# INDA23PlusPlus/isaklm-raytracer

Measured on AMD Instinct MI355X. Metric: Msamples/sec (W×H×spp/s) at 1920×1080; achieved HBM GB/s vs peak, higher is better.
Workload: dtype f32

## Files before the change

### isaklm-raytracer_amd/csrc/wavefront.hip

```cpp
#include <hip/hip_runtime.h>

#include <stdio.h>
#include <stdlib.h>
#include <string.h>
#include <time.h>

#include <algorithm>
#include <chrono>
#include <atomic>
#include <map>
#include <mutex>
#include <thread>
#include <vector>

#include "bvh_trace.h"
#include "rt_kernels.h"

using namespace rtk;

#define WF_BLOCK 256
#ifndef WF_TBLOCK
#define WF_TBLOCK 256
#endif
static_assert(WF_BLOCK % WF_TBLOCK == 0 && WF_TBLOCK % 64 == 0, "WF_TBLOCK must divide WF_BLOCK in whole waves");
// ... 1561 lines not shown
    uint32_t *fetch = st.counts + 4;
    const int limit = fr.max_depth > 0 ? fr.max_depth : RT_WATCHDOG_BOUNCES;

    PathRegs p;
    p.slot = 0;
    p.ro = p.rd = rt_v3(0, 0, 0);
    CoopRay r;
    coop_idle(r);
    int hit = -1;
    float bx = 0.0f, by = 0.0f, bz = 0.0f;
    bool active = false;
    bool exhausted = lane >= ppw;
    bool pending = false;
    while (true) {
        const bool need = !active && !exhausted;
        const unsigned long long m = __ballot(need);
        if (m) {
            const int leader = __ffsll((long long)m) - 1;
            uint32_t base = 0;
            if (lane == leader) base = atomicAdd(fetch, (uint32_t)__popcll(m));
            base = __shfl(base, leader);
            if (need) {
                const uint32_t e = base + (uint32_t)__popcll(m & ((1ull << lane) - 1ull));
                if (e >= n) {
                    exhausted = true;
                } else {
                    active = true;
                    first_ray(st, fr, st.q_slot[q][e], p);
                    if (COUNT) c.v[RT_CNT_RAY]++;
                    if (!coop_begin(sc, r, p.ro, p.rd)) {
                        pending = true;
                        hit = -1;
                    }
                }
            }
        }
        while (pending) {
            pending = false;
            if (shade_step<COUNT>(sc, fr, cam, p, hit, bx, by, bz, limit, c)) {
                if (COUNT) c.v[RT_CNT_RAY]++;
                if (!coop_begin(sc, r, p.ro, p.rd)) {
                    pending = true;
                    hit = -1;
                }
            } else {
                store_regs(st, fr, p);
                active = false;
            }
        }
        const unsigned long long lm = __ballot(r.live);
        if (!lm) {
            if (__all(exhausted)) break;
            continue;
        }
        if (__popcll(lm) <= wide) {
            const WideLds W{s_wide + wave * WIDE_CAP, WIDE_CAP, wkey, reinterpret_cast<float *>(wkey + 1), w.mark};
            for (unsigned long long mm = lm; mm; mm &= mm - 1) {
                const int owner = __ffsll((long long)mm) - 1;
                const int ot = wave * 64 + owner;
                const Stack<WF_LDS_STACK> so{s_node + ot, s_entry + ot, WF_BLOCK,
                                             st.spill + blockIdx.x * WF_BLOCK + ot, st.spill_threads};
                int t;
                float x, y, z;
                wide_resume<COUNT>(sc, r, owner, so, W, t, x, y, z, c);
                if (lane == owner) {
                    hit = t;
                    bx = x;
                    by = y;
                    bz = z;
                    r.live = false;
                    pending = true;
                }
            }
            continue;
        }
        if (coop_round<COUNT>(sc, r, stk, w, cap, postpone, hit, bx, by, bz, c)) pending = true;
    }
    if (COUNT) {
        flush_counters(c, fr.counters);
        flush_finish_counters(c, fr.counters);
    }
}

template <bool COUNT>
__global__ void __launch_bounds__(WF_BLOCK, WF_LONG_WAVES) wf_long(RtDevScene sc, RtDevFrame fr, RtDevCamera cam, WfState st,
                                                    int final_slice)
{
    __shared__ __attribute__((aligned(16))) WideItem s_wide[(WF_BLOCK / 64) * WIDE_CAP];
    static_assert(WSM_LDS_BYTES <= WIDE_CAP * sizeof(WideItem), "the wide s_min query's lists reuse the wave's frontier");
    static_assert(WSM_KD_STACK * 8 <= 128 * sizeof(int), "the bounded KD phase's stack reuses the wave's chunk_owner marks");
    __shared__ unsigned long long s_key[(WF_BLOCK / 64) * 4];
    __shared__ __attribute__((aligned(8))) int s_mark[2 * WF_BLOCK];
    if (WF_LONG_PRIO > 0) __builtin_amdgcn_s_setprio(WF_LONG_PRIO);
    const int lane = __lane_id();
    const int wave = threadIdx.x >> 6;
    const WideLds W{s_wide + wave * WIDE_CAP, WIDE_CAP, s_key + wave * 4,
                    reinterpret_cast<float *>(s_key + wave * 4 + 1), s_mark + wave * 128};
    Cnt c;
    if (COUNT) c.zero();
    const int limit = fr.max_depth > 0 ? fr.max_depth : RT_WATCHDOG_BOUNCES;
    uint32_t *const reserved = st.long_ctr, *const claimed = st.long_ctr + 1, *const running = st.long_ctr + 3;
    const bool persist = st.fin_live != nullptr;
    unsigned long long t_idle = __builtin_amdgcn_s_memrealtime();
    unsigned long long t_net = t_idle;
    unsigned long long t_pub = 0;
    uint32_t n_idle = 0, n_net = 0, n_pub = 0, n_start = 0;
    uint32_t r_seen = 0, e_pub = 0xffffffffu;
    while (true) {
        uint32_t e = 0, slot = 0;
        RtF4 ro4{0, 0, 0, 0}, rd4{0, 0, 0, 0};
        int quit = 0;
        if (lane == 0) {
            while (true) {
                const unsigned long long now = __builtin_amdgcn_s_memrealtime();
                ++n_idle;
                ++n_net;
                const uint32_t fl = persist ? __hip_atomic_load(st.fin_live, __ATOMIC_RELAXED, __HIP_MEMORY_SCOPE_AGENT) : 0u;
                const bool unstarted = persist && !(fl & WF_FIN_STARTED);
                const bool producing = persist && !unstarted && (fl & ~WF_FIN_STARTED) != 0u;
                const bool others = __hip_atomic_load(running, __ATOMIC_RELAXED, __HIP_MEMORY_SCOPE_AGENT) != 0u;
                const bool chain_open =
                    persist && __hip_atomic_load(st.chain_flag, __ATOMIC_RELAXED, __HIP_MEMORY_SCOPE_AGENT) != 0u;
                if (persist && !producing && !unstarted) __builtin_amdgcn_fence(__ATOMIC_ACQUIRE, "agent");
                e = __hip_atomic_load(claimed, __ATOMIC_RELAXED, __HIP_MEMORY_SCOPE_AGENT);
                const uint32_t rw = __hip_atomic_load(reserved, __ATOMIC_RELAXED, __HIP_MEMORY_SCOPE_AGENT);
                const bool closed = (rw & WF_LONG_CLOSED) != 0u;
                const uint32_t r = rw & ~WF_LONG_CLOSED;
                const bool flowing = r != r_seen;
                if (flowing) {
                    r_seen = r;
                    t_idle = now;
                    n_idle = 0;
                }
                if (flowing || producing || others) {
                    t_net = now;
                    n_net = 0;
                }
                const bool window_over = (now - t_idle > WF_LONG_CHAIN_IDLE || n_idle > WF_LONG_CHAIN_TRIPS) && !others;
                const bool done = persist && (closed || (!producing && !unstarted && (!chain_open || window_over)));
                if (st.debug_quit) {
                    quit = 2;
                    break;
                }
                if (e < r) {
                    const uint32_t k = e % st.long_cap;
                    const unsigned long long v =
                        __hip_atomic_load(st.long_ent + k, __ATOMIC_RELAXED, __HIP_MEMORY_SCOPE_AGENT);
                    if ((uint32_t)(v >> 32) == e + 1u) {
                        __builtin_amdgcn_fence(__ATOMIC_ACQUIRE, "agent");
                        ro4 = ldf4(st.long_ray + 2 * (size_t)k);
                        rd4 = ldf4(st.long_ray + 2 * (size_t)k + 1);
                        slot = (uint32_t)v;
                        asm volatile("s_waitcnt vmcnt(0)" ::: "memory");
                        uint32_t expect = e;
                        if (__hip_atomic_compare_exchange_strong(claimed, &expect, e + 1u, __ATOMIC_RELAXED,
                                                                 __ATOMIC_RELAXED, __HIP_MEMORY_SCOPE_AGENT)) {
                            __hip_atomic_fetch_add(running, 1u, __ATOMIC_RELAXED, __HIP_MEMORY_SCOPE_AGENT);
                            break;
                        }
                        continue;
                    }
                    if (e != e_pub) {
                        e_pub = e;
                        t_pub = now;
                        n_pub = 0;
                    } else if (now - t_pub > WF_LONG_PUBLISH_WAIT || ++n_pub > WF_LONG_PUBLISH_TRIPS) {
                        quit = 2;
                        break;
                    }
                } else {
                    if (persist ? done : (final_slice || !others)) {
                        quit = 1;
                        break;
                    }
                    if (unstarted && !closed && ++n_start > WF_LONG_START_TRIPS) {
                        uint32_t x = r;
                        if (__hip_atomic_compare_exchange_strong(reserved, &x, r | WF_LONG_CLOSED, __ATOMIC_RELAXED,
                                                                 __ATOMIC_RELAXED, __HIP_MEMORY_SCOPE_AGENT)) {
                            atomicAdd(fr.dev_stats + RT_DEV_LONG_CLOSED, 1ull);
                            quit = 1;
                            break;
                        }
                        continue;
                    }
                }
                if (now - t_net > WF_LONG_IDLE || n_net > WF_LONG_IDLE_TRIPS) {
                    quit = e < r ? 2 : 1;
                    break;
                }
                __builtin_amdgcn_s_sleep(16);
            }
            if (!quit) asm volatile("s_waitcnt vmcnt(0)" ::: "memory");
            if (quit == 2) atomicAdd(fr.dev_stats + RT_DEV_LONG_QUIT, 1ull);
        }
        if (__builtin_amdgcn_readfirstlane(quit)) break;
        e = (uint32_t)__builtin_amdgcn_readfirstlane((int)e);
        PathRegs p;
        p.slot = 0;
        p.ro = p.rd = rt_v3(0, 0, 0);
        if (lane == 0) {
            load_regs(st, fr, slot, p);
            p.ro = ld3(ro4);
            p.rd = ld3(rd4);
        }
        int want = 0;
        uint32_t ret_e = 0;
        const unsigned long long t_claim = __builtin_amdgcn_s_memrealtime();
        uint32_t bounces = 0;
        while (true) {
            ++bounces;
            int hit = -1;
            float bx = 0.0f, by = 0.0f, bz = 0.0f;
            CoopRay r;
            coop_idle(r);
            if (lane == 0) {
                if (COUNT) c.v[RT_CNT_RAY]++;
                coop_begin(sc, r, p.ro, p.rd);
            }
            if (__shfl((int)r.live, 0)) {
                const Vec3D o = rt_v3(__shfl(r.o.x, 0), __shfl(r.o.y, 0), __shfl(r.o.z, 0));
                const Vec3D d = rt_v3(__shfl(r.d.x, 0), __shfl(r.d.y, 0), __shfl(r.d.z, 0));
                const float en = __shfl(r.entry, 0), ex = __shfl(r.exit_, 0);
                bool traced = false;
                bool certified = false;
                if (st.long_wide && rt_bounded_ray(o, d, sc.split_vals, sc.split_off)) {
                    float s_min = ex;
                    int tk = -1;
                    traced = wide_smin<COUNT>(sc, o, d, ex, wsm_lds(W.F, W.key, st.long_wide == 2), s_min, tk, c);
                    if (traced && s_min < ex)
                        certified = kd_certified<COUNT>(sc, o, d, en, ex, s_min, tk, hit, bx, by, bz, c, lane == 0);
                    if (traced && s_min < ex && !certified) {
                        LdsStack1 ks{reinterpret_cast<uint2 *>(W.mark)};
                        const int tstar = tk >= 0 ? (int)sc.bvh_bary[tk].tri : -1;
                        hit = kd_bounded_wave<COUNT>(sc, o, d, en, ex, s_min, tstar, bx, by, bz, ks,
                                                     reinterpret_cast<unsigned long long *>(W.F), c);
                    }
                    if (!traced && lane == 0) atomicAdd(fr.dev_stats + RT_DEV_WIDE_OVERFLOW, 1ull);
                }
                if (!traced) {
                    const int nf = !COUNT && sc.kd_grid > 0 ? kd_origin_frontier(sc, o, d, en, ex, W) : 0;
                    if (nf > 0) wide_trace_from<COUNT>(sc, o, d, nf, W, lane == 0, hit, bx, by, bz, c);
                    else wide_trace<COUNT>(sc, o, d, en, ex, W, lane == 0, hit, bx, by, bz, c);
                }
                if (COUNT && lane == 0 && hit >= 0 && !certified) c.cert[1]++;
            }
            want = 0;
            if (lane == 0) {
                want = shade_step<COUNT>(sc, fr, cam, p, hit, bx, by, bz, limit, c) ? 1 : 0;
                if (!want && st.long_return) {
                    while (true) {
                        store_regs(st, fr, p);
                        asm volatile("s_waitcnt vmcnt(0)" ::: "memory");
                        __builtin_amdgcn_fence(__ATOMIC_RELEASE, "agent");
                        uint32_t x = RT_PX_OUT;
                        if (__hip_atomic_compare_exchange_strong(st.pxo + p.slot, &x, RT_PX_LONGDONE, __ATOMIC_RELAXED,
                                                                 __ATOMIC_RELAXED, __HIP_MEMORY_SCOPE_AGENT))
                            break;
                        x = __hip_atomic_exchange(st.pxo + p.slot, RT_PX_OUT, __ATOMIC_RELAXED,
                                                  __HIP_MEMORY_SCOPE_AGENT);
                        p.passes_left = (int)(x & RT_PX_PASSES);
                        if (x & RT_PX_PASSES) {
                            atomicAdd(fr.dev_stats + RT_DEV_OWED_PIXELS, 1ull);
                            atomicAdd(fr.dev_stats + RT_DEV_OWED_PASSES, (unsigned long long)(x & RT_PX_PASSES));
                        }
                        const Vec3D fb = fr.fb[p.slot];
                        const float sq = fr.sq[p.slot];
                        const int count = fr.count[p.slot];
                        if (start_sample<COUNT>(fr, cam, (int)p.slot, p.passes_left, p.rng, fb, sq, count, p.ro, p.rd,
                                                c)) {
                            p.T = rt_v3(1.0f, 1.0f, 1.0f);
                            p.L = rt_v3(0.0f, 0.0f, 0.0f);
                            p.inside = false;
                            p.prev_type = PRIMARY;
                            p.depth = 1;
                            p.shadow = false;
                            want = 1;
                            break;
                        }
                    }
                }
                if (want && st.long_return && p.depth == 1 && !p.shadow) {
                    unsigned long long *const ret_word = reinterpret_cast<unsigned long long *>(st.ret_ctr);
                    if (st.linger == 0ull &&
                        __hip_atomic_load(st.chain_flag, __ATOMIC_RELAXED, __HIP_MEMORY_SCOPE_AGENT) != 0u) {
                        want = 2;
                        ret_e = (uint32_t)__hip_atomic_fetch_add(ret_word, 1ull, __ATOMIC_RELAXED, __HIP_MEMORY_SCOPE_AGENT);
                    }
                    unsigned long long w = __hip_atomic_load(ret_word, __ATOMIC_RELAXED, __HIP_MEMORY_SCOPE_AGENT);
                    while (want != 2 && (w >> 32) != 0ull) {
                        if (__hip_atomic_compare_exchange_strong(ret_word, &w, w + 1ull, __ATOMIC_RELAXED,
                                                                 __ATOMIC_RELAXED, __HIP_MEMORY_SCOPE_AGENT)) {
                            want = 2;
                            ret_e = (uint32_t)w;
                            break;
                        }
                    }
                }
            }
            want = __builtin_amdgcn_readfirstlane(want);
            if (want != 1) break;
        }
        if (lane == 0) {
            if (st.long_log && e < 65535u) {
                unsigned long long *L = st.long_log + 4 + 4 * (size_t)e;
                L[0] = t_claim;
                L[1] = __builtin_amdgcn_s_memrealtime();
                L[2] = bounces;
                L[3] = p.slot;
            }
            if (want == 2) {
                store_regs(st, fr, p);
                st.ro[p.slot] = p.ro;
                st.cont[p.slot] = p.rd;
                asm volatile("s_waitcnt vmcnt(0)" ::: "memory");
                __builtin_amdgcn_fence(__ATOMIC_RELEASE, "agent");
                asm volatile("s_waitcnt vmcnt(0)" ::: "memory");
                __hip_atomic_store(st.ret_ring + ret_e % st.long_cap, ((unsigned long long)(ret_e + 1u) << 32) | p.slot,
                                   __ATOMIC_RELAXED, __HIP_MEMORY_SCOPE_AGENT);
            } else if (st.long_return) {
                __hip_atomic_fetch_sub(st.ret_ctr + 3, 1u, __ATOMIC_RELAXED, __HIP_MEMORY_SCOPE_AGENT);
            } else {
                store_regs(st, fr, p);
            }
            __hip_atomic_fetch_sub(running, 1u, __ATOMIC_RELAXED, __HIP_MEMORY_SCOPE_AGENT);
        }
        t_idle = __builtin_amdgcn_s_memrealtime();
        n_idle = 0;
    }
    if (COUNT) {
        flush_counters(c, fr.counters);
        flush_cert_counters(c, fr.dev_stats);
    }
}

void rt_register_shutdown();

namespace {

struct Pipe {
    std::vector<std::pair<float, float>> trace_iv;
    WfState st{};
    hipStream_t stream = nullptr;
    uint32_t *host_count = nullptr;
    hipEvent_t ev[6] = {};
    hipEvent_t join = nullptr;
    hipEvent_t fin_done = nullptr;
    hipEvent_t long_done = nullptr;
    bool joined = false;
    bool long_rec = false;
    RtProfile prof{};
};

struct ChainKey {
    const void *nodes, *bvh, *fb, *sq, *count, *rng;
    int width, height, adaptive, min_samples, max_depth, shard_id, num_shards, long_depth;
    float tolerance;
    RtDevCamera cam;
};

ChainKey chain_key(const RtDevScene &sc, const RtDevFrame &fr, const RtDevCamera &cam, int long_depth)
{
    ChainKey key;
    memset(&key, 0, sizeof key);
    key.nodes = sc.nodes;
    key.bvh = sc.bvh_nodes;
    key.fb = fr.fb;
    key.sq = fr.sq;
    key.count = fr.count;
    key.rng = fr.rng;
    key.width = fr.width;
    key.height = fr.height;
    key.adaptive = fr.adaptive;
    key.min_samples = fr.min_samples;
    key.max_depth = fr.max_depth;
    key.shard_id = fr.shard_id;
    key.num_shards = fr.num_shards;
    key.long_depth = long_depth;
    key.tolerance = fr.tolerance;
    key.cam = cam;
    return key;
}

struct Pending {
    bool on = false;
    int dev = 0;
    RtDevScene sc{};
    RtDevFrame fr{};
    RtDevCamera cam{};
    hipStream_t stream = nullptr;
    int long_depth = 0, debug = 0, calls = 0;
    bool prof = false;
    uint32_t check_mask = 0;
    ChainKey key{};
};

struct Workspace {
    Pending pend;
    size_t slots = 0;
    int grid = 0;
    int spill_pipes = 0;
    void *blob = nullptr;
    Pipe pipe[WF_MAX_PIPES];
    bool streams_ok = false;
    hipEvent_t fork = nullptr, ev0 = nullptr, ev1 = nullptr, fin_ready = nullptr;
    hipEvent_t long_ev = nullptr;
    bool recorded = false;
    uint32_t *fin_live = nullptr;
    uint32_t *heavy_list = nullptr;
    RtF4 *chk = nullptr;
    uint32_t chk_cap = 0;
    uint32_t *chk_ctr = nullptr;
    uint32_t *verify_res = nullptr;
    bool verify_pending = false;
    bool verify_unread = false;
    hipEvent_t verify_ev = nullptr;
// ... 177 lines not shown
        st.cont = (Vec3D *)(b + o_c);
        st.snorm = (Vec3D *)(b + o_n);
        st.rp = (Vec3D *)(b + o_rp);
        st.light = (int *)(b + o_li);
        st.ro = (Vec3D *)(b + o_ro);
        st.e_sh = (uint32_t *)(b + o_es);
        st.e_ext = (uint32_t *)(b + o_ee);
        st.q_slot[0] = (uint32_t *)(b + o_qs0[i]);
        st.q_slot[1] = (uint32_t *)(b + o_qs1[i]);
        st.q_ray[0] = (RtF4 *)(b + o_qr0[i]);
        st.q_ray[1] = (RtF4 *)(b + o_qr1[i]);
        st.hits = (RtF4 *)(b + o_h[i]);
        st.counts = (uint32_t *)(b + o_cnt[i]);
        st.spill = i < spill_pipes ? (uint2 *)(b + o_sp[i]) : nullptr;
        st.spill_threads = (int)spill_threads;
        st.long_ctr = (uint32_t *)(b + o_lc);
        st.long_ent = (unsigned long long *)(b + o_le);
        st.long_ray = (RtF4 *)(b + o_lr);
        st.long_depth = 0;
        st.long_cap = (uint32_t)slots;
        st.long_return = 0;
        st.ret_ring = (unsigned long long *)(b + o_rr);
        st.ret_ctr = (uint32_t *)(b + o_rc);
        st.linger = WF_FIN_LINGER;
        st.pxo = (uint32_t *)(b + o_px);
        st.heavy = (uint8_t *)(b + o_hv);
        st.listed = (uint32_t *)(b + o_ls);
        st.heavy_list = nullptr;
        w.heavy_list = (uint32_t *)(b + o_hl);
        st.heavy_n = (uint32_t *)(b + o_hn);
        st.fin_live = nullptr;
        st.chain_flag = (uint32_t *)(b + o_ctl + 128);
        st.fresh = 0;
        st.fresh_n = 0;
        st.span = nullptr;
        st.call_id = 0;
        st.chk = nullptr;
        st.chk_ctr = nullptr;
        st.chk_mask = 0;
        st.chk_cap = 0;
        st.chk_fault = 0;
        st.debug_quit = 0;
        st.long_wide = 0;
    }
    w.slots = slots;
    w.grid = grid;
    w.spill_pipes = spill_pipes;
    return 0;
}

float elapsed_ms(hipEvent_t a, hipEvent_t b)
{
    float ms = 0.0f;
    return hipEventElapsedTime(&ms, a, b) == hipSuccess ? ms : 0.0f;
}

int launch_verify(Workspace &w, hipStream_t stream)
{
    if (!w.verify_pending || !w.blob) return 0;
    w.verify_pending = false;
    const int blocks = (int)std::min<size_t>((w.slots + WF_BLOCK - 1) / WF_BLOCK, 1024);
    hipLaunchKernelGGL(wf_verify, dim3(blocks), dim3(WF_BLOCK), 0, stream, w.pipe[0].st, (uint32_t)w.slots,
                       w.verify_res, w.last_fr.dev_stats);
    if (hipGetLastError() != hipSuccess) return -1;
    if (hipEventRecord(w.verify_ev, stream) != hipSuccess) return -1;
    w.verify_rec = true;
    w.verify_unread = true;
    return 0;
}

int join_all(Workspace &w, hipStream_t stream)
{
    if (launch_drain(w) != 0) return -1;
    if (w.verify_rec && hipStreamWaitEvent(stream, w.verify_ev, 0) != hipSuccess) return -1;
    for (int pi = 0; pi < WF_MAX_PIPES; ++pi) {
        Pipe &p = w.pipe[pi];
        if (p.joined && hipStreamWaitEvent(stream, p.join, 0) != hipSuccess) return -1;
        if (p.long_rec && hipStreamWaitEvent(stream, p.long_done, 0) != hipSuccess) return -1;
    }
    if (w.recorded && hipStreamWaitEvent(stream, w.long_ev, 0) != hipSuccess) return -1;
    return launch_verify(w, stream);
}

int debug_long_log(Workspace &w, unsigned long long *buf);

int launch_whole_now(Workspace &w, int dev, const RtDevScene &sc, const RtDevFrame &fr, const RtDevCamera &cam,
                     hipStream_t stream, int long_depth, bool prof, bool overlap, uint32_t check_mask, int debug,
                     bool count)
{
    const size_t slots = (size_t)fr.width * fr.height;
    overlap = overlap && !fr.reset;
    if (!w.cus) {
        hipDeviceProp_t prop;
        w.cus = hipGetDeviceProperties(&prop, dev) == hipSuccess && prop.multiProcessorCount > 0
                    ? prop.multiProcessorCount
                    : 256;
    }
    const int grid = w.cus * 4 * WF_FIN_BVH_WAVES / (WF_BLOCK / 64);
    const ChainKey key = chain_key(sc, fr, cam, long_depth);
    const bool chained = overlap && w.chain_open && !fr.reset && memcmp(&key, &w.key, sizeof key) == 0;
    if (!chained && join_all(w, stream) != 0) return -1;
    if (ensure(w, slots, grid, 1) != 0) return -1;
    Pipe &pp = w.pipe[0];
    WfState st = pp.st;
    const int long_return = long_depth > 0 ? 1 : 0;
    st.long_depth = long_depth;
    st.long_return = long_return;
    st.fresh = 1;
    st.fresh_n = (uint32_t)(((fr.width + 15) / 16) * ((fr.height + 15) / 16)) * 256u;
    st.linger = overlap ? 0ull : WF_FIN_LINGER;
    st.chk_mask = check_mask;
    const int par = (int)(w.call_seq & 1);
    if (check_mask != 0xFFFFFFFFu) {
        const unsigned long long per_sample =
            check_mask == 0u ? 2ull * (unsigned long long)(long_depth > 0 ? long_depth : RT_DEEP_PATH) + 2ull : 8ull;
        const unsigned long long want = (unsigned long long)slots * (unsigned long long)fr.passes * per_sample /
                                        ((unsigned long long)check_mask + 1ull);
        uint32_t cap = 1u << 16;
        while (cap < want && cap < WF_CHECK_CAP) cap <<= 1;
        if (cap > w.chk_cap) {
            if (w.chk) {
                if (hipDeviceSynchronize() != hipSuccess) return -1;
                (void)hipFree(w.chk);
                w.chk = nullptr;
                w.chk_cap = 0;
            }
            if (hipMalloc((void **)&w.chk, 2 * (size_t)cap * 3 * sizeof(RtF4)) != hipSuccess) {
                w.chk = nullptr;
                return -1;
            }
            w.chk_cap = cap;
        }
    }
    st.chk = check_mask == 0xFFFFFFFFu ? nullptr : w.chk + 3 * (size_t)w.chk_cap * (size_t)par;
    st.chk_cap = w.chk_cap;
    st.chk_ctr = w.chk_ctr + par;
    st.chk_fault = (debug & RT_DEBUG_CHECK_FAULT) ? 1 : 0;
    st.debug_quit = (debug & RT_DEBUG_LONG_QUIT) ? 1 : 0;
    st.long_wide = sc.bvh_wide ? ((debug & RT_DEBUG_WIDE_CAP1) ? 2 : 1) : 0;
    if ((debug & RT_DEBUG_LONG_LOG) && !w.long_log_buf &&
        hipMalloc((void **)&w.long_log_buf, 8 * 4 * 65536) != hipSuccess) {
        w.long_log_buf = nullptr;
        return -1;
    }
    unsigned long long *const long_log_buf = w.long_log_buf;
    st.long_log = (debug & RT_DEBUG_LONG_LOG) ? long_log_buf : nullptr;
    int fgrid = (int)((slots + WF_BLOCK - 1) / WF_BLOCK);
    const int fmax = long_return ? grid - WF_LONG_BLOCKS : grid;
    fgrid = fgrid > fmax ? fmax : fgrid;
    const uint32_t k = (uint32_t)(w.call_seq % 8);
    st.fin_live = long_return ? w.fin_live + k : nullptr;
    st.call_id = (uint32_t)w.call_seq + 1u;
    if (!chained) {
        if (long_return) {
            if (hipMemsetAsync(st.long_ctr, 0, 256, stream) != hipSuccess) return -1;
            if (hipMemsetAsync(st.long_ent, 0, (size_t)st.long_cap * 8, stream) != hipSuccess) return -1;
            if (hipMemsetAsync(st.ret_ring, 0, (size_t)st.long_cap * 8, stream) != hipSuccess) return -1;
            if (hipMemsetAsync(st.ret_ctr, 0, 256, stream) != hipSuccess) return -1;
        }
        if (st.long_log && hipMemsetAsync(long_log_buf, 0, 8 * 4 * 65536, stream) != hipSuccess) return -1;
    }
    ++w.call_seq;
    const hipStream_t s = pp.stream;
    if (hipEventRecord(w.fork, stream) != hipSuccess || hipStreamWaitEvent(s, w.fork, 0) != hipSuccess) return -1;
    if (hipMemsetAsync(st.counts, 0, 256, s) != hipSuccess) return -1;
    if (st.fin_live && hipMemsetD32Async((hipDeviceptr_t)st.fin_live, (int)(fgrid * (WF_BLOCK / 64)), 1, s) != hipSuccess)
        return -1;
    if (st.chk) {
        if (w.chk_rec[par] && hipStreamWaitEvent(s, w.chk_done[par], 0) != hipSuccess) return -1;
        if (hipMemsetAsync(st.chk_ctr, 0, 4, s) != hipSuccess) return -1;
    }
    if (long_return && hipMemsetD32Async((hipDeviceptr_t)st.chain_flag, overlap ? 1 : 0, 1, s) != hipSuccess) return -1;
    st.span = nullptr;
    if (prof) {
        if (prof_slot(w, s, &st.span, fr.passes) != 0) return -1;
    }
    st.heavy_list = nullptr;
    if (long_return && w.heavy_list && WF_HEAVY_FIRST) {
        st.heavy_list = w.heavy_list;
        if (hipMemsetAsync(st.heavy_n, 0, 4, s) != hipSuccess) return -1;
        hipLaunchKernelGGL(wf_heavy_list, dim3(WF_HEAVY_BLOCKS), dim3(WF_BLOCK), 0, s, fr, st, st.call_id,
                           (uint32_t)WF_HEAVY_SPLIT, 256u);
        hipLaunchKernelGGL(wf_heavy_list, dim3(WF_HEAVY_BLOCKS), dim3(WF_BLOCK), 0, s, fr, st, st.call_id, 1u,
                           (uint32_t)WF_HEAVY_SPLIT);
        if (hipGetLastError() != hipSuccess) return -1;
    }
    if (hipEventRecord(w.fin_ready, s) != hipSuccess) return -1;
    Pipe *lp = long_return ? &w.pipe[1] : nullptr;
    const bool long_first = lp && (debug & RT_DEBUG_SERIAL_LONG_FIRST);
    const bool fin_first = lp && !long_first && (debug & RT_DEBUG_SERIAL_FIN_FIRST);
    auto launch_long = [&]() -> int {
        if (hipStreamWaitEvent(lp->stream, fin_first ? pp.fin_done : w.fin_ready, 0) != hipSuccess) return -1;
        if (count) hipLaunchKernelGGL(wf_long<true>, dim3(WF_LONG_BLOCKS), dim3(WF_BLOCK), 0, lp->stream, sc, fr, cam, st, 1);
        else hipLaunchKernelGGL(wf_long<false>, dim3(WF_LONG_BLOCKS), dim3(WF_BLOCK), 0, lp->stream, sc, fr, cam, st, 1);
        if (hipGetLastError() != hipSuccess) return -1;
        if (hipEventRecord(lp->long_done, lp->stream) != hipSuccess) return -1;
        lp->long_rec = true;
        return 0;
    };
    if (long_first && (launch_long() != 0 || hipStreamWaitEvent(s, lp->long_done, 0) != hipSuccess)) return -1;
    if (count && !(debug & RT_DEBUG_COUNT_LONG_ONLY)) hipLaunchKernelGGL(wf_finish_bvh<true>, dim3(fgrid), dim3(WF_BLOCK), 0, s, sc, fr, cam, st, 0);
    else if (fgrid <= w.cus * WF_FIN_SMALL_WAVES)
        hipLaunchKernelGGL((wf_finish_bvh<false, 1>), dim3(fgrid), dim3(WF_BLOCK), 0, s, sc, fr, cam, st, 0);
    else hipLaunchKernelGGL(wf_finish_bvh<false>, dim3(fgrid), dim3(WF_BLOCK), 0, s, sc, fr, cam, st, 0);
    if (hipGetLastError() != hipSuccess) return -1;
    if (hipEventRecord(pp.fin_done, s) != hipSuccess) return -1;
    if (lp && !long_first && launch_long() != 0) return -1;
    if (st.chk) {
        Pipe &cp = w.pipe[2];
        WfState cs = st;
        cs.spill = cp.st.spill;
        if (!cs.spill) return -1;
        if (hipStreamWaitEvent(cp.stream, pp.fin_done, 0) != hipSuccess) return -1;
        hipLaunchKernelGGL(wf_check, dim3(WF_CHECK_BLOCKS), dim3(WF_BLOCK), 0, cp.stream, sc, cs, fr.dev_stats);
        if (hipGetLastError() != hipSuccess) return -1;
        if (hipEventRecord(w.chk_done[par], cp.stream) != hipSuccess || hipEventRecord(cp.join, cp.stream) != hipSuccess)
            return -1;
        w.chk_rec[par] = true;
        cp.joined = true;
    }
    if (hipEventRecord(pp.join, s) != hipSuccess) return -1;
    pp.joined = true;
    if (!overlap) {
        if (hipStreamWaitEvent(stream, pp.join, 0) != hipSuccess) return -1;
        if (lp && hipStreamWaitEvent(stream, lp->long_done, 0) != hipSuccess) return -1;
    }
    w.chain_open = overlap && long_return;
    w.verify_pending = w.verify_pending || long_return;
    w.key = key;
    w.last_sc = sc;
    w.last_fr = fr;
    w.last_fr.reset = 0;
    w.last_cam = cam;
    w.last_long_depth = long_depth;
    w.last_debug = debug;
    if (debug & RT_DEBUG_CALL_LOG) {
        (void)hipStreamSynchronize(s);
        timespec ts;
        clock_gettime(CLOCK_MONOTONIC, &ts);
        uint32_t lc[4] = {}, rc4[7] = {};
        (void)hipMemcpy(lc, st.long_ctr, sizeof lc, hipMemcpyDeviceToHost);
        (void)hipMemcpy(rc4, st.ret_ctr, sizeof rc4, hipMemcpyDeviceToHost);
        fprintf(stderr,
                "[wf] call %llu%s finisher done t %.4f; long entries %u claimed %u running %u; returns reserved %u "
                "claimed %u, finisher waves alive %u, pixels out %u; owed passes: most %u, pixels %u\n",
                w.call_seq, chained ? " (chained)" : "", ts.tv_sec + ts.tv_nsec * 1e-9, lc[0], lc[1], lc[3], rc4[0],
                rc4[2], rc4[1], rc4[3], rc4[5], rc4[6]);
    }
    if (st.long_log && !overlap) return debug_long_log(w, long_log_buf);
    return 0;
}

int flush_pending(Workspace &w)
{
    if (!w.pend.on) return 0;
    Pending b = w.pend;
    w.pend.on = false;
    return launch_whole_now(w, b.dev, b.sc, b.fr, b.cam, b.stream, b.long_depth, b.prof, true, b.check_mask, b.debug,
                            false);
}

int launch_whole(Workspace &w, int dev, const RtDevScene &sc, const RtDevFrame &fr, const RtDevCamera &cam,
                 hipStream_t stream, int long_depth, bool prof, bool overlap, uint32_t check_mask, int debug,
                 bool count, int coalesce)
{
    const bool can = overlap && !fr.reset && !count && coalesce > 0 && !fr.wave_times &&
                     !(debug & (RT_DEBUG_CALL_LOG | RT_DEBUG_LONG_LOG | RT_DEBUG_SERIAL_LONG_FIRST |
                                RT_DEBUG_SERIAL_FIN_FIRST));
    if (w.pend.on) {
        const ChainKey key = chain_key(sc, fr, cam, long_depth);
        if (can && w.pend.dev == dev && w.pend.stream == stream && w.pend.prof == prof &&
            w.pend.check_mask == check_mask && w.pend.debug == debug && w.pend.sc.nodes == sc.nodes &&
            memcmp(&key, &w.pend.key, sizeof key) == 0 && (long long)w.pend.fr.passes + fr.passes < (1LL << 28)) {
            w.pend.fr.passes += fr.passes;
            ++w.pend.calls;
            return w.pend.fr.passes < coalesce ? 0 : flush_pending(w);
        }
        if (flush_pending(w) != 0) return -1;
    }
    if (can && fr.passes < coalesce) {
        Pending &b = w.pend;
        b.on = true;
        b.dev = dev;
        b.sc = sc;
        b.fr = fr;
        b.cam = cam;
        b.stream = stream;
        b.long_depth = long_depth;
        b.debug = debug;
        b.calls = 1;
        b.prof = prof;
        b.check_mask = check_mask;
        b.key = chain_key(sc, fr, cam, long_depth);
        return 0;
    }
    return launch_whole_now(w, dev, sc, fr, cam, stream, long_depth, prof, overlap, check_mask, debug, count);
}

int launch_drain(Workspace &w)
{
    if (flush_pending(w) != 0) return -1;
    if (!w.chain_open) return 0;
    w.chain_open = false;
    const RtDevFrame &fr = w.last_fr;
    const size_t slots = (size_t)fr.width * fr.height;
    Pipe &pp = w.pipe[0];
    WfState st = pp.st;
    st.long_depth = w.last_long_depth;
    st.long_return = 1;
    st.fresh = 1;
    st.fresh_n = 0;
    st.span = nullptr;
    st.linger = WF_FIN_LINGER;
    st.chk = nullptr;
    st.chk_mask = 0;
    st.chk_ctr = w.chk_ctr;
    st.chk_fault = 0;
    st.debug_quit = (w.last_debug & RT_DEBUG_LONG_QUIT) ? 1 : 0;
    st.long_wide = w.last_sc.bvh_wide ? ((w.last_debug & RT_DEBUG_WIDE_CAP1) ? 2 : 1) : 0;
    st.long_log = nullptr;
    int fgrid = (int)((slots + WF_BLOCK - 1) / WF_BLOCK);
    fgrid = fgrid > w.grid - WF_LONG_BLOCKS ? w.grid - WF_LONG_BLOCKS : fgrid;
    st.fin_live = w.fin_live + (uint32_t)(w.call_seq % 8);
    ++w.call_seq;
    const hipStream_t s = pp.stream;
    if (hipMemsetAsync(st.counts, 0, 256, s) != hipSuccess) return -1;
    if (hipMemsetAsync(st.ret_ctr + 4, 0, 4, s) != hipSuccess) return -1;
    if (hipMemsetAsync(st.chain_flag, 0, 4, s) != hipSuccess) return -1;
    if (hipMemsetD32Async((hipDeviceptr_t)st.fin_live, (int)(fgrid * (WF_BLOCK / 64)), 1, s) != hipSuccess) return -1;
    if (hipEventRecord(w.fin_ready, s) != hipSuccess) return -1;
    if (fgrid <= w.cus * WF_FIN_SMALL_WAVES)
        hipLaunchKernelGGL((wf_finish_bvh<false, 1>), dim3(fgrid), dim3(WF_BLOCK), 0, s, w.last_sc, fr, w.last_cam, st, 0);
    else hipLaunchKernelGGL(wf_finish_bvh<false>, dim3(fgrid), dim3(WF_BLOCK), 0, s, w.last_sc, fr, w.last_cam, st, 0);
    if (hipGetLastError() != hipSuccess) return -1;
    Pipe &lp = w.pipe[1];
    if (hipStreamWaitEvent(lp.stream, w.fin_ready, 0) != hipSuccess) return -1;
    hipLaunchKernelGGL(wf_long<false>, dim3(WF_LONG_BLOCKS), dim3(WF_BLOCK), 0, lp.stream, w.last_sc, fr, w.last_cam, st, 1);
    if (hipGetLastError() != hipSuccess) return -1;
    if (hipEventRecord(lp.long_done, lp.stream) != hipSuccess) return -1;
    lp.long_rec = true;
    if (hipEventRecord(pp.join, s) != hipSuccess) return -1;
    pp.joined = true;
    w.verify_pending = true;
    if (w.last_debug & RT_DEBUG_CALL_LOG) {
        (void)hipStreamSynchronize(s);
        timespec ts;
        clock_gettime(CLOCK_MONOTONIC, &ts);
        uint32_t rc[7] = {};
        (void)hipMemcpy(rc, st.ret_ctr, sizeof rc, hipMemcpyDeviceToHost);
        fprintf(stderr, "[wf] drain done t %.4f; returns reserved %u claimed %u, pixels out %u; owed passes: most %u, pixels %u\n",
                ts.tv_sec + ts.tv_nsec * 1e-9, rc[0], rc[2], rc[3], rc[5], rc[6]);
    }
    return 0;
}

int debug_long_log(Workspace &w, unsigned long long *buf)
{
    (void)w;
    (void)hipDeviceSynchronize();
    std::vector<unsigned long long> L(4 * 65536);
    (void)hipMemcpy(L.data(), buf, 8 * L.size(), hipMemcpyDeviceToHost);
    struct Rec { double start, end; unsigned long long bounces, slot; };
    std::vector<Rec> v;
    double last = 0;
    for (size_t e = 1; e < 65536; ++e)
        if (L[4 * e + 1]) {
            v.push_back({(L[4 * e] - L[0]) * 1e-5, (L[4 * e + 1] - L[0]) * 1e-5, L[4 * e + 2], L[4 * e + 3]});
            last = std::max(last, v.back().end);
        }
    std::sort(v.begin(), v.end(), [](const Rec &a, const Rec &b) { return a.end > b.end; });
    fprintf(stderr, "[wf long log] %zu deep samples, last end %.1f ms; latest 12 (start ms, end ms, bounces, us/bounce, slot):\n",
            v.size(), last);
    for (size_t i = 0; i < v.size() && i < 12; ++i)
        fprintf(stderr, "  %.1f %.1f %llu %.2f %llu\n", v[i].start, v[i].end, v[i].bounces,
                (v[i].end - v[i].start) * 1e3 / (double)(v[i].bounces ? v[i].bounces : 1), v[i].slot);
    std::sort(v.begin(), v.end(), [](const Rec &a, const Rec &b) { return a.bounces > b.bounces; });
    fprintf(stderr, "[wf long log] longest 8:\n");
    for (size_t i = 0; i < v.size() && i < 8; ++i)
        fprintf(stderr, "  %.1f %.1f %llu %.2f %llu\n", v[i].start, v[i].end, v[i].bounces,
                (v[i].end - v[i].start) * 1e3 / (double)(v[i].bounces ? v[i].bounces : 1), v[i].slot);
    std::map<unsigned long long, Rec> px;
    std::map<unsigned long long, int> nd;
    for (const Rec &r : v) {
        auto it = px.find(r.slot);
        if (it == px.end()) {
            px[r.slot] = Rec{r.start, r.end, 0, (unsigned long long)0};
            it = px.find(r.slot);
        }
        it->second.start = std::min(it->second.start, r.start);
        it->second.end = std::max(it->second.end, r.end);
        it->second.slot += (unsigned long long)((r.end - r.start) * 1e3);
        it->second.bounces += r.bounces;
        ++nd[r.slot];
    }
    std::vector<std::pair<unsigned long long, Rec>> pv(px.begin(), px.end());
    std::sort(pv.begin(), pv.end(), [](const auto &a, const auto &b) { return a.second.end > b.second.end; });
    fprintf(stderr, "[wf long log] %zu pixels; latest-ending 10 (slot, deep samples, bounces, ms in wf_long, first claim, last end):\n",
            pv.size());
    for (size_t i = 0; i < pv.size() && i < 10; ++i)
        fprintf(stderr, "  %llu %d %llu %.1f %.1f %.1f\n", pv[i].first, nd[pv[i].first], pv[i].second.bounces,
                pv[i].second.slot * 1e-3, pv[i].second.start, pv[i].second.end);
    return 0;
}

}

int rt_wavefront_device_init()
{
    int dev = 0;
    if (hipGetDevice(&dev) != hipSuccess) return -1;
    rt_register_shutdown();
    return ensure_streams(workspace(dev), WF_PIPES_DEFAULT);
}

static thread_local char g_incomplete[256];

const char *rt_wavefront_incomplete_msg() { return g_incomplete; }

int rt_wavefront_join(void *stream, int consume)
{
    int dev = 0;
    if (hipGetDevice(&dev) != hipSuccess) return -1;
    Workspace *w = nullptr;
    {
        std::lock_guard<std::mutex> g(g_ws_mu);
        auto it = g_ws.find(dev);
        if (it == g_ws.end() || !it->second) return 0;
        w = it->second;
    }
    if (stream) return join_all(*w, (hipStream_t)stream);
    if (launch_drain(*w) != 0) return -1;
    for (int pi = 0; pi < WF_MAX_PIPES; ++pi) {
        Pipe &p = w->pipe[pi];
        if (p.joined && hipEventSynchronize(p.join) != hipSuccess) return -1;
        if (p.long_rec && hipEventSynchronize(p.long_done) != hipSuccess) return -1;
    }
    if (w->recorded && hipEventSynchronize(w->long_ev) != hipSuccess) return -1;
    if (w->verify_pending) {
        const hipStream_t s = w->pipe[0].stream;
        if (launch_verify(*w, s) != 0) return -1;
    }
    if (w->verify_rec && hipEventSynchronize(w->verify_ev) != hipSuccess) return -1;
    if (!w->verify_unread) return 0;
    uint32_t r[5] = {};
    if (hipMemcpy(r, w->verify_res, sizeof r, hipMemcpyDeviceToHost) != hipSuccess) return -1;
    if (!consume) return 0;
    w->verify_unread = false;
    if (hipMemset(w->verify_res, 0, sizeof r) != hipSuccess || hipDeviceSynchronize() != hipSuccess) return -1;
    if (r[0] | r[1] | r[2] | r[3] | r[4]) {
        snprintf(g_incomplete, sizeof g_incomplete,
                 "%u pixels stranded in the deep-path hand-off (pixels out %u, returns unclaimed %u, hand-offs "
                 "unclaimed %u, finisher waves registered %u): the frame misses passes; RtDeviations counts it",
                 r[0], r[1], r[2], r[3], r[4]);
// ... 365 lines not shown
```

### isaklm-raytracer_amd/csrc/wide_bvh.h

```cpp
#pragma once
#include "bvh_trace.h"
#include "wide_bvh_caps.h"

namespace rtk {

#define WSM_KD_STACK 32
#define WSM_LDS_BYTES (2 * WSM_FCAP * 4 + 2 * WSM_LCAP * 4)

typedef __attribute__((address_space(3))) volatile uint32_t lds_vu32;

struct WsmLds {
    uint32_t *F;
    uint32_t *L;
    unsigned long long *key;
    int fcap, lcap;
};

struct LdsStack1 {
    uint2 *s;
    __device__ __forceinline__ void put(int k, uint32_t node, float t) { s[k] = make_uint2(node, __float_as_uint(t)); }
    __device__ __forceinline__ void get(int k, uint32_t &node, float &entry) const
    {
        const uint2 v = s[k];
        node = v.x;
        entry = __uint_as_float(v.y);
    }
    __device__ __forceinline__ uint32_t node_at(int k) const { return s[k].x; }
    __device__ __forceinline__ float entry_at(int k) const { return __uint_as_float(s[k].y); }
};

__device__ __forceinline__ WsmLds wsm_lds(void *bytes, unsigned long long *key, int cap1)
{
    uint32_t *f = reinterpret_cast<uint32_t *>(bytes);
    uint32_t *l = f + 2 * WSM_FCAP;
    return WsmLds{f, l, key, cap1 ? 1 : WSM_FCAP, cap1 ? 1 : WSM_LCAP};
}
template <bool COUNT>
__device__ __forceinline__ bool wide_smin(const RtDevScene &sc, Vec3D o, Vec3D d, float best0, const WsmLds &W,
                                          float &best_out, int &tk_out, Cnt &c)
{
    constexpr int A = RT_BVHW_ARITY;
    const int lane = __lane_id();
    const RtSlab sl = rt_slab(o, d, rt_ray_margin(o.x, o.y, o.z, sc.bvh_scale));
    lds_vu64 *vkey = (lds_vu64 *)W.key;
    lds_vu32 *F = (lds_vu32 *)W.F;
    lds_vu32 *L = (lds_vu32 *)W.L;
    if (lane == 0) {
        vkey[0] = ~0ull;
        vkey[1] = ~0ull;
        F[0] = 0u;
    }
    int n = 1, nl = 0, cur = 0;
    float best = best0;
    bool have = false;
    if (COUNT && lane == 0) c.v[RT_CNT_WIDE_CALLS]++;
    while (n > 0 || nl > 0) {
        if (COUNT && lane == 0) c.v[RT_CNT_WIDE_ROUNDS]++;
        lds_vu32 *Fc = F + cur * WSM_FCAP, *Fn = F + (cur ^ 1) * WSM_FCAP;
        lds_vu32 *Lc = L + cur * WSM_LCAP, *Ln = L + (cur ^ 1) * WSM_LCAP;
        const int pairs = n * A, tests = nl * 8;
        int nn = 0, nln = 0;
        for (int base = 0; base < pairs || base < tests; base += 64) {
            const int p = base + lane;
            const bool ev = p < pairs;
            const uint32_t it = Fc[ev ? p / A : 0];
            const bool lv0 = p < tests;
            const uint32_t lref = Lc[lv0 ? p >> 3 : 0];
            const RtF4 *rec = sc.bvh_wide + 2 * ((size_t)(ev ? it : 0u) * A + (size_t)(p % A));
            const RtF4 r0 = ldf4(rec), r1 = ldf4(rec + 1);
            const bool lv = lv0 && (uint32_t)(p & 7) <= (lref & 7u);
            const uint32_t slot = lv ? ((lref & ~RT_BVH_LEAF) >> 3) + (uint32_t)(p & 7) : 0u;
            const RtF4 P = ldf4(sc.bvh_a + slot);
            const RtIsectBary *br = sc.bvh_bary + slot;
            const RtF4 B = ldf4(&br->b), C = ldf4(&br->c), D = ldf4(&br->d);
            const float rd = __uint_as_float(br->rd);
            asm volatile("" ::"v"(r0.x), "v"(r1.x), "v"(P.x), "v"(B.x), "v"(C.x), "v"(D.x), "v"(rd));
            const uint32_t ref = __float_as_uint(r1.z);
            float tn;
            const bool hit = rt_bvh_box(r0.x, r0.y, r0.z, r0.w, r1.x, r1.y, sl, best, tn) && ev && ref != RT_BVH_EMPTY;
            const bool inner = hit && !(ref & RT_BVH_LEAF), leaf = hit && (ref & RT_BVH_LEAF);
            const unsigned long long mi = __ballot(inner), ml = __ballot(leaf);
            const int pi = nn + (int)__builtin_amdgcn_mbcnt_hi((uint32_t)(mi >> 32), __builtin_amdgcn_mbcnt_lo((uint32_t)mi, 0u));
            const int pl = nln + (int)__builtin_amdgcn_mbcnt_hi((uint32_t)(ml >> 32), __builtin_amdgcn_mbcnt_lo((uint32_t)ml, 0u));
            if (inner && pi < W.fcap) Fn[pi] = ref;
            if (leaf && pl < W.lcap) Ln[pl] = ref;
            nn += __popcll(mi);
            nln += __popcll(ml);
            float s;
            const bool plane = lv && rt_tri_plane(P, o, d, INFINITY, s) && (s < best || (s == best && have));
            if (COUNT) {
                const unsigned long long mn = __ballot(ev && p % A == 0), mt = __ballot(lv), mb = __ballot(plane);
                if (lane == 0) {
                    c.v[RT_CNT_B_BVH_NODE] += (unsigned long long)__popcll(mn);
                    c.v[RT_CNT_B_BVH_TRI] += (unsigned long long)__popcll(mt);
                    c.v[RT_CNT_B_BARY] += (unsigned long long)__popcll(mb);
                }
            }
            if (plane) {
                float cx, cy, cz;
                if (rt_tri_bary(B, C, D, rd, o, d, s, cx, cy, cz)) {
                    const uint32_t sb = __float_as_uint(s);
                    const unsigned long long old = atomicMin(W.key, (unsigned long long)sb << 32 | slot);
                    if ((uint32_t)(old >> 32) == sb) atomicMin(reinterpret_cast<uint32_t *>(W.key + 1), sb);
                }
            }
        }
        if (nn > W.fcap || nln > W.lcap) return false;
        const unsigned long long key = vkey[0];
        have = key != ~0ull;
        if (have) best = __uint_as_float((uint32_t)(key >> 32));
        n = nn;
        nl = nln;
        cur ^= 1;
    }
    const unsigned long long key = vkey[0], tie = vkey[1];
    best_out = best;
    tk_out = !have ? -1 : ((uint32_t)tie == (uint32_t)(key >> 32) ? RT_TK_TIE : (int)(uint32_t)key);
    return true;
}

#define WSM_KD_BLOCK 64

template <bool COUNT, typename STACK>
__device__ __forceinline__ int kd_bounded_wave(const RtDevScene &sc, const Vec3D o, const Vec3D d, float entry,
                                               const float root_exit, const float s_min, const int tstar, float &hbx,
                                               float &hby, float &hbz, STACK &stk, unsigned long long *block, Cnt &c)
{
    const int lane = __lane_id();
    lds_vu64 *blk = (lds_vu64 *)block;
    uint32_t base = 0xFFFFFFFFu;
    const uint32_t last = (uint32_t)sc.node_count - 1u;
    auto fetch = [&](uint32_t node) -> uint2 {
        if (COUNT && lane == 0) c.v[RT_CNT_NODE]++;
        if (node - base >= (uint32_t)WSM_KD_BLOCK || base == 0xFFFFFFFFu) {
            base = node;
            const uint32_t k = node + (uint32_t)lane;
            const uint2 v = ldc_u2(sc.nodes + 2 * (size_t)(k < last ? k : last));
            blk[lane] = (unsigned long long)v.y << 32 | v.x;
        }
        const unsigned long long v = blk[node - base];
// ... 87 lines not shown
```

Before: 875.7.

## Keep long-path state in LDS and add optional phase timing stamps

Several fields of the per-wave path state in the long-path kernel (slot, light, hit point, continuation and shading normal) now live in LDS through proxy wrapper types instead of registers. The aim is to cut VGPR pressure in wf_long and allow more waves. The change also adds phase timing instrumentation behind a compile flag, sizes the check buffer and check grid differently, and replaces a device-wide synchronize with per-event waits. The volatile LDS accesses add latency on each use of those fields.

After: 865.0. -1.2%, worse.

```diff
diff --git a/isaklm-raytracer_amd/csrc/wavefront.hip b/isaklm-raytracer_amd/csrc/wavefront.hip
--- a/isaklm-raytracer_amd/csrc/wavefront.hip
+++ b/isaklm-raytracer_amd/csrc/wavefront.hip
@@ -1667,6 +1667,60 @@
     }
 }
 
+#define WF_DEV_PHASE 37
+#define WF_DEV_PHASES 8
+static_assert(WF_DEV_PHASE > RT_DEV_CERT_FALLBACK && WF_DEV_PHASE + WF_DEV_PHASES <= RT_DEV_WORDS,
+              "the phase sums use spare words of the deviation statistics");
+#ifdef WF_LONG_STAMPS
+#define WF_STAMP(k)                                                                                                  \
+    do {                                                                                                             \
+        asm volatile("s_waitcnt vmcnt(0) lgkmcnt(0)" ::: "memory");                                                  \
+        const unsigned long long t_ = __builtin_amdgcn_s_memtime();                                                  \
+        ph[k] += t_ - t_ph;                                                                                          \
+        t_ph = t_;                                                                                                   \
+    } while (0)
+#else
+#define WF_STAMP(k) \
+    do {            \
+    } while (0)
+#endif
+#define WF_LONG_LDS 12
+typedef __attribute__((address_space(3))) volatile float lds_vf32;
+typedef __attribute__((address_space(3))) volatile uint32_t lds_vw32;
+struct LongLdsV3 {
+    lds_vf32 *w;
+    __device__ __forceinline__ operator Vec3D() const { return rt_v3(w[0], w[1], w[2]); }
+    __device__ __forceinline__ LongLdsV3 &operator=(Vec3D v)
+    {
+        w[0] = v.x;
+        w[1] = v.y;
+        w[2] = v.z;
+        return *this;
+    }
+    __device__ __forceinline__ LongLdsV3 &operator=(const LongLdsV3 &o) { return *this = (Vec3D)o; }
+};
+template <typename T>
+struct LongLdsWord {
+    lds_vw32 *w;
+    __device__ __forceinline__ operator T() const { return (T)*w; }
+    __device__ __forceinline__ LongLdsWord &operator=(T v)
+    {
+        *w = (uint32_t)v;
+        return *this;
+    }
+    __device__ __forceinline__ LongLdsWord &operator=(const LongLdsWord &o) { return *this = (T)o; }
+};
+struct PathRegsW {
+    LongLdsWord<uint32_t> slot;
+    bool shadow, inside, dual, ext_live;
+    int prev_type, depth, passes_left;
+    LongLdsWord<int> light;
+    uint32_t rng;
+    Vec3D T, L;
+    LongLdsV3 rp, cont, snorm;
+    Vec3D ro, rd;
+};
+
 template <bool COUNT>
 __global__ void __launch_bounds__(WF_BLOCK, WF_LONG_WAVES) wf_long(RtDevScene sc, RtDevFrame fr, RtDevCamera cam, WfState st,
                                                     int final_slice)
@@ -1676,6 +1730,7 @@
     static_assert(WSM_KD_STACK * 8 <= 128 * sizeof(int), "the bounded KD phase's stack reuses the wave's chunk_owner marks");
     __shared__ unsigned long long s_key[(WF_BLOCK / 64) * 4];
     __shared__ __attribute__((aligned(8))) int s_mark[2 * WF_BLOCK];
+    __shared__ uint32_t s_path[(WF_BLOCK / 64) * WF_LONG_LDS];
     if (WF_LONG_PRIO > 0) __builtin_amdgcn_s_setprio(WF_LONG_PRIO);
     const int lane = __lane_id();
     const int wave = threadIdx.x >> 6;
@@ -1683,6 +1738,10 @@
                     reinterpret_cast<float *>(s_key + wave * 4 + 1), s_mark + wave * 128};
     Cnt c;
     if (COUNT) c.zero();
+#ifdef WF_LONG_STAMPS
+    unsigned long long ph[WF_DEV_PHASES] = {0, 0, 0, 0, 0, 0, 0, 0}, t_ph = 0;
+    uint32_t smin_rounds = 0;
+#endif
     const int limit = fr.max_depth > 0 ? fr.max_depth : RT_WATCHDOG_BOUNCES;
     uint32_t *const reserved = st.long_ctr, *const claimed = st.long_ctr + 1, *const running = st.long_ctr + 3;
     const bool persist = st.fin_live != nullptr;
@@ -1780,9 +1839,10 @@
         }
         if (__builtin_amdgcn_readfirstlane(quit)) break;
         e = (uint32_t)__builtin_amdgcn_readfirstlane((int)e);
-        PathRegs p;
-        p.slot = 0;
-        p.ro = p.rd = rt_v3(0, 0, 0);
+        lds_vw32 *const pw = (lds_vw32 *)(s_path + wave * WF_LONG_LDS);
+        lds_vf32 *const pf = (lds_vf32 *)(s_path + wave * WF_LONG_LDS);
+        PathRegsW p{{pw},     false,    false,    false,          false,         PRIMARY, 0, 0, {pw + 1}, 0u, rt_v3(0, 0, 0),
+                    rt_v3(0, 0, 0), {pf + 2}, {pf + 5}, {pf + 8}, rt_v3(0, 0, 0), rt_v3(0, 0, 0)};
         if (lane == 0) {
             load_regs(st, fr, slot, p);
             p.ro = ld3(ro4);
@@ -1792,6 +1852,10 @@
         uint32_t ret_e = 0;
         const unsigned long long t_claim = __builtin_amdgcn_s_memrealtime();
         uint32_t bounces = 0;
+#ifdef WF_LONG_STAMPS
+        asm volatile("s_waitcnt vmcnt(0) lgkmcnt(0)" ::: "memory");
+        t_ph = __builtin_amdgcn_s_memtime();
+#endif
         while (true) {
             ++bounces;
             int hit = -1;
@@ -1806,14 +1870,21 @@
                 const Vec3D o = rt_v3(__shfl(r.o.x, 0), __shfl(r.o.y, 0), __shfl(r.o.z, 0));
                 const Vec3D d = rt_v3(__shfl(r.d.x, 0), __shfl(r.d.y, 0), __shfl(r.d.z, 0));
                 const float en = __shfl(r.entry, 0), ex = __shfl(r.exit_, 0);
+                WF_STAMP(2);
                 bool traced = false;
                 bool certified = false;
                 if (st.long_wide && rt_bounded_ray(o, d, sc.split_vals, sc.split_off)) {
                     float s_min = ex;
                     int tk = -1;
+#ifdef WF_LONG_STAMPS
+                    traced = wide_smin<COUNT>(sc, o, d, ex, wsm_lds(W.F, W.key, st.long_wide == 2), s_min, tk, c, &smin_rounds);
+#else
                     traced = wide_smin<COUNT>(sc, o, d, ex, wsm_lds(W.F, W.key, st.long_wide == 2), s_min, tk, c);
+#endif
+                    WF_STAMP(3);
                     if (traced && s_min < ex)
                         certified = kd_certified<COUNT>(sc, o, d, en, ex, s_min, tk, hit, bx, by, bz, c, lane == 0);
+                    WF_STAMP(4);
                     if (traced && s_min < ex && !certified) {
                         LdsStack1 ks{reinterpret_cast<uint2 *>(W.mark)};
                         const int tstar = tk >= 0 ? (int)sc.bvh_bary[tk].tri : -1;
@@ -1828,10 +1899,18 @@
                     else wide_trace<COUNT>(sc, o, d, en, ex, W, lane == 0, hit, bx, by, bz, c);
                 }
                 if (COUNT && lane == 0 && hit >= 0 && !certified) c.cert[1]++;
+                WF_STAMP(5);
             }
             want = 0;
+#ifdef WF_LONG_STAMPS
+            unsigned long long t_shade = 0;
+#endif
             if (lane == 0) {
                 want = shade_step<COUNT>(sc, fr, cam, p, hit, bx, by, bz, limit, c) ? 1 : 0;
+#ifdef WF_LONG_STAMPS
+                asm volatile("s_waitcnt vmcnt(0) lgkmcnt(0)" ::: "memory");
+                t_shade = __builtin_amdgcn_s_memtime();
+#endif
                 if (!want && st.long_return) {
                     while (true) {
                         store_regs(st, fr, p);
@@ -1883,8 +1962,20 @@
                 }
             }
             want = __builtin_amdgcn_readfirstlane(want);
+#ifdef WF_LONG_STAMPS
+            {
+                const unsigned long long t_ = (unsigned long long)(uint32_t)__builtin_amdgcn_readfirstlane((int)(uint32_t)t_shade) |
+                                              (unsigned long long)(uint32_t)__builtin_amdgcn_readfirstlane((int)(uint32_t)(t_shade >> 32)) << 32;
+                ph[6] += t_ - t_ph;
+                t_ph = t_;
+            }
+#endif
+            WF_STAMP(7);
             if (want != 1) break;
         }
+#ifdef WF_LONG_STAMPS
+        ph[0] += bounces;
+#endif
         if (lane == 0) {
             if (st.long_log && e < 65535u) {
                 unsigned long long *L = st.long_log + 4 + 4 * (size_t)e;
@@ -1916,6 +2007,12 @@
         flush_counters(c, fr.counters);
         flush_cert_counters(c, fr.dev_stats);
     }
+#ifdef WF_LONG_STAMPS
+    ph[1] = smin_rounds;
+    if (lane == 0)
+        for (int k = 0; k < WF_DEV_PHASES; ++k)
+            if (ph[k]) atomicAdd(fr.dev_stats + WF_DEV_PHASE + k, ph[k]);
+#endif
 }
 
 void rt_register_shutdown();
@@ -2259,7 +2356,7 @@
     return launch_verify(w, stream);
 }
 
-int debug_long_log(Workspace &w, unsigned long long *buf);
+int debug_long_log(Workspace &w, unsigned long long *buf, const unsigned long long *dev_stats);
 
 int launch_whole_now(Workspace &w, int dev, const RtDevScene &sc, const RtDevFrame &fr, const RtDevCamera &cam,
                      hipStream_t stream, int long_depth, bool prof, bool overlap, uint32_t check_mask, int debug,
@@ -2291,13 +2388,15 @@
     if (check_mask != 0xFFFFFFFFu) {
         const unsigned long long per_sample =
             check_mask == 0u ? 2ull * (unsigned long long)(long_depth > 0 ? long_depth : RT_DEEP_PATH) + 2ull : 8ull;
-        const unsigned long long want = (unsigned long long)slots * (unsigned long long)fr.passes * per_sample /
-                                        ((unsigned long long)check_mask + 1ull);
+        const unsigned long long want = long_return ? (unsigned long long)slots * (unsigned long long)fr.passes *
+                                                          per_sample / ((unsigned long long)check_mask + 1ull)
+                                                    : (unsigned long long)WF_CHECK_CAP;
         uint32_t cap = 1u << 16;
         while (cap < want && cap < WF_CHECK_CAP) cap <<= 1;
         if (cap > w.chk_cap) {
             if (w.chk) {
-                if (hipDeviceSynchronize() != hipSuccess) return -1;
+                for (int i = 0; i < 2; ++i)
+                    if (w.chk_rec[i] && hipEventSynchronize(w.chk_done[i]) != hipSuccess) return -1;
                 (void)hipFree(w.chk);
                 w.chk = nullptr;
                 w.chk_cap = 0;
@@ -2389,7 +2488,8 @@
         cs.spill = cp.st.spill;
         if (!cs.spill) return -1;
         if (hipStreamWaitEvent(cp.stream, pp.fin_done, 0) != hipSuccess) return -1;
-        hipLaunchKernelGGL(wf_check, dim3(WF_CHECK_BLOCKS), dim3(WF_BLOCK), 0, cp.stream, sc, cs, fr.dev_stats);
+        const int cgrid = overlap ? (WF_CHECK_BLOCKS < w.grid ? WF_CHECK_BLOCKS : w.grid) : grid;
+        hipLaunchKernelGGL(wf_check, dim3(cgrid), dim3(WF_BLOCK), 0, cp.stream, sc, cs, fr.dev_stats);
         if (hipGetLastError() != hipSuccess) return -1;
         if (hipEventRecord(w.chk_done[par], cp.stream) != hipSuccess || hipEventRecord(cp.join, cp.stream) != hipSuccess)
             return -1;
@@ -2424,7 +2524,7 @@
                 w.call_seq, chained ? " (chained)" : "", ts.tv_sec + ts.tv_nsec * 1e-9, lc[0], lc[1], lc[3], rc4[0],
                 rc4[2], rc4[1], rc4[3], rc4[5], rc4[6]);
     }
-    if (st.long_log && !overlap) return debug_long_log(w, long_log_buf);
+    if (st.long_log && !overlap) return debug_long_log(w, long_log_buf, fr.dev_stats);
     return 0;
 }
 
@@ -2531,9 +2631,10 @@
     return 0;
 }
 
-int debug_long_log(Workspace &w, unsigned long long *buf)
+int debug_long_log(Workspace &w, unsigned long long *buf, const unsigned long long *dev_stats)
 {
     (void)w;
+    (void)dev_stats;
     (void)hipDeviceSynchronize();
     std::vector<unsigned long long> L(4 * 65536);
     (void)hipMemcpy(L.data(), buf, 8 * L.size(), hipMemcpyDeviceToHost);
@@ -2546,6 +2647,20 @@
             last = std::max(last, v.back().end);
         }
     std::sort(v.begin(), v.end(), [](const Rec &a, const Rec &b) { return a.end > b.end; });
+#ifdef WF_LONG_STAMPS
+    {
+        unsigned long long ph[WF_DEV_PHASES] = {};
+        (void)hipMemcpy(ph, dev_stats + WF_DEV_PHASE, sizeof ph, hipMemcpyDeviceToHost);
+        const double nb = (double)(ph[0] ? ph[0] : 1);
+        unsigned long long sum = 0;
+        for (int k = 2; k < WF_DEV_PHASES; ++k) sum += ph[k];
+        fprintf(stderr,
+                "[wf long phases] %llu bounces, %.2f wide_smin rounds each; cycles per bounce %.0f: set-up and broadcast "
+                "%.0f, wide_smin %.0f, kd_certified %.0f, cold traversals %.0f, shade_step %.0f, pixel bookkeeping %.0f\n",
+                ph[0], (double)ph[1] / nb, (double)sum / nb, (double)ph[2] / nb, (double)ph[3] / nb, (double)ph[4] / nb,
+                (double)ph[5] / nb, (double)ph[6] / nb, (double)ph[7] / nb);
+    }
+#endif
     fprintf(stderr, "[wf long log] %zu deep samples, last end %.1f ms; latest 12 (start ms, end ms, bounces, us/bounce, slot):\n",
             v.size(), last);
     for (size_t i = 0; i < v.size() && i < 12; ++i)
diff --git a/isaklm-raytracer_amd/csrc/wide_bvh.h b/isaklm-raytracer_amd/csrc/wide_bvh.h
--- a/isaklm-raytracer_amd/csrc/wide_bvh.h
+++ b/isaklm-raytracer_amd/csrc/wide_bvh.h
@@ -37,7 +37,7 @@
 }
 template <bool COUNT>
 __device__ __forceinline__ bool wide_smin(const RtDevScene &sc, Vec3D o, Vec3D d, float best0, const WsmLds &W,
-                                          float &best_out, int &tk_out, Cnt &c)
+                                          float &best_out, int &tk_out, Cnt &c, uint32_t *rounds = nullptr)
 {
     constexpr int A = RT_BVHW_ARITY;
     const int lane = __lane_id();
@@ -56,6 +56,7 @@
     if (COUNT && lane == 0) c.v[RT_CNT_WIDE_CALLS]++;
     while (n > 0 || nl > 0) {
         if (COUNT && lane == 0) c.v[RT_CNT_WIDE_ROUNDS]++;
+        if (rounds) ++*rounds;
         lds_vu32 *Fc = F + cur * WSM_FCAP, *Fn = F + (cur ^ 1) * WSM_FCAP;
         lds_vu32 *Lc = L + cur * WSM_LCAP, *Ln = L + (cur ^ 1) * WSM_LCAP;
         const int pairs = n * A, tests = nl * 8;
```
